# Kim-Dongjun/Soft-Truncation

Measured on AMD Instinct MI355X. Metric: training images/sec (DDPM++ CIFAR-10 32x32), higher is better.
Workload: dtype f32; 1 GPU; DDPM++ (VP) CIFAR-10 32x32, configs/vp/CIFAR10/ddpmpp_nll_st.py (BASELINE configs[1]); per_gpu_batch=128, global_batch=128, parallelism=dp1

## Files before the change

soft-truncation_amd/csrc/conv.hip:

```cpp
#include "igemm.h"
#include "split.h"
#include "stk_fp16.h"
#include "stk_fp16_train.h"

namespace {

using igemm::Cfg;
using igemm::MnMajor;
using igemm::keep_if;
using igemm::strip_row;

typedef __attribute__((address_space(1))) float gfloat;

struct ConvP {
  const float* x1; const float* x2; int C1, C2;
  const float* w; int w_layout;
  const float* bias; const float* temb; int temb_stride; const float* res; float inv_div; int use_div;
  float* y;
  const float* dy; float* dx1; float* dx2; float beta1, beta2, alpha;
  float* part; long part_stride;
  int N, H, W, Cin, Cout, OH, OW, KH, KW, stride, pad, sshift;
  int HW, OHW, taps;
  int ohw_shift, ow_shift;
};
// ... 920 lines not shown
    using A2 = std::conditional_t<X1, x2::ActLoader16<true, TAPS>, x2::ActLoader<true, TAPS>>;
    if (g.dual) hipLaunchKernelGGL((x2::gemm_kernel<A2, E>), g.grid, dim3(256), 0, g.s, g.p, g.q, g.M, g.Ng, g.tm, g.tn, g.nch,
                                   g.chunks_per_split, g.xpart, g.nx);
    else hipLaunchKernelGGL((x2::gemm_kernel<A1, E>), g.grid, dim3(256), 0, g.s, g.p, g.q, g.M, g.Ng, g.tm, g.tn, g.nch,
                            g.chunks_per_split, g.xpart, g.nx);
  } else if (g.halo) {
    if (g.p.W == 64)
      hipLaunchKernelGGL((x2d::gemm_halo_kernel<64, E, 1>), g.grid, dim3(256), 0, g.s, g.p, g.q, g.M, g.Ng, g.tm, g.tn, g.nch / 9, g.xpart, g.nx);
    else if (g.p.W == 32)
      hipLaunchKernelGGL((x2d::gemm_halo_kernel<32, E, 1>), g.grid, dim3(256), 0, g.s, g.p, g.q, g.M, g.Ng, g.tm, g.tn, g.nch / 9, g.xpart, g.nx);
    else
      hipLaunchKernelGGL((x2d::gemm_halo_kernel<16, E, 1>), g.grid, dim3(256), 0, g.s, g.p, g.q, g.M, g.Ng, g.tm, g.tn, g.nch / 9, g.xpart, g.nx);
  } else {
    hipLaunchKernelGGL((x2d::gemm_kernel<TAPS, 128, E>), g.grid, dim3(256), 0, g.s, g.p, g.q, g.M, g.Ng, g.tm, g.tn, g.nch,
                       g.chunks_per_split, g.xpart, g.nx);
  }
}
template <class E>
void split_gemm(const SplitGemm& g) {
  if (g.p.taps == 9) split_gemm_taps<E, 9>(g);
  else split_gemm_taps<E, 1>(g);
}

template <class EP>
int launch_split(ConvP p, const SplitPlan& r0, const float* s1, int S1, const float* s2, int S2, int M, long Ng, int dgrad,
                 void* ws, hipStream_t s, const void* wp_ready, float* amax, const void* planes, const float* planes_amax,
                 bool amax_valid, bool x1) {
  x2::Src q;
  q.s1 = s1; q.s2 = S2 > 0 ? s2 : s1; q.S1 = S1; q.S2 = S2; q.Kc = S1 + S2; q.Mpad = x2::pad128(M); q.taps = p.taps;
  q.pl = static_cast<const unsigned char*>(planes); q.pl_stride = planes ? pl::plane_bytes(p.N, S1, p.HW) : 0;
  const SplitWs lay = split_ws(r0, M, q.Kc, p.taps);
  unsigned char* base = reinterpret_cast<unsigned char*>(((uintptr_t)ws + 255) & ~(uintptr_t)255);
  float* xpart = reinterpret_cast<float*>(base + lay.xpart);
  p.part = reinterpret_cast<float*>(base + lay.part);
  p.part_stride = r0.slab;
  if (amax) xpart = amax + (dgrad ? 2 * x2::NPART : 0);
  if (planes) {
    xpart = const_cast<float*>(planes_amax);
  } else if (!(amax_valid && amax)) {
    hipLaunchKernelGGL(x2::amax_partial_kernel, dim3(x2::NPART), dim3(x2::AMAX_THREADS), 0, s, s1, (long)p.N * S1 * p.HW, xpart);
    if (S2 > 0)
      hipLaunchKernelGGL(x2::amax_partial_kernel, dim3(x2::NPART), dim3(x2::AMAX_THREADS), 0, s, s2, (long)p.N * S2 * p.HW,
                         xpart + x2::NPART);
    STK_CHECK_LAUNCH();
  }
  if (wp_ready) {
    q.wp = static_cast<const unsigned short*>(wp_ready);
  } else {
    x2::WprepDesc one = {};
    one.w = p.w; one.wp = base; one.M = M; one.Kc = q.Kc; one.Mpad = q.Mpad;
    one.taps = p.taps; one.flip = dgrad;
    split_weight_strides(p, dgrad, one.sm, one.sk);
    hipLaunchKernelGGL(x2::wamax_kernel, dim3(x2::WPART, 1), dim3(256), 0, s, nullptr, one);
    hipLaunchKernelGGL(x2::wprep_kernel, dim3((unsigned)stk_cdiv((long)q.Mpad * q.Kc, 256L)), dim3(256), 0, s, nullptr, one);
    STK_CHECK_LAUNCH();
    q.wp = reinterpret_cast<const unsigned short*>(base);
  }
  const int nch = planes && x1 ? p.taps * ((q.Kc / x2::KC + 1) / 2) : p.taps * (q.Kc / x2::KC);
  const SplitPlan r = planes && x1 ? x1_plan(r0, nch) : r0;
  SplitGemm g = {p, q, M, (int)Ng, q.Mpad / 128, stk_cdiv((int)Ng, 128), nch, r.chunks_per_split, xpart,
                 S2 > 0 ? 2 * x2::NPART : x2::NPART, S2 > 0, planes != nullptr, planes && x2d::halo_ok(p, p.taps, r0.splits),
                 dim3(), s};
  g.grid = dim3((unsigned)(g.tm * g.tn * r.splits));
  if (r0.splits == 1) {
    if (x1) split_gemm<OneProduct<EP>>(g);
    else split_gemm<EP>(g);
    STK_CHECK_LAUNCH();
    return STK_OK;
  }
  if (x1) split_gemm<OneProduct<EpSlab>>(g);
  else split_gemm<EpSlab>(g);
  STK_CHECK_LAUNCH();
  launch_slab_sum(p, r.splits, M, Ng, dgrad, s);
  STK_CHECK_LAUNCH();
  return STK_OK;
}

struct SplitWgradPlan { int ok; int splits; int chunks_per_split; long slab; int rows3; };
inline SplitWgradPlan split_wgrad_plan(int C1, int C2, int N, int Cout, int H, int W, int OH, int OW, int KH, int KW,
                                       int stride, int pad) {
  SplitWgradPlan q = {0, 0, 0, 0, 0};
  const int Cin = C1 + C2;
  const long K = (long)N * H * W;
  const int cmax = Cout > C1 ? (Cout > C2 ? Cout : C2) : (C1 > C2 ? C1 : C2);
  if (K * cmax * 4 >= 0x7fffffffL || (C2 > 0 && C1 % 32)) return q;
  const bool pow2 = (W & (W - 1)) == 0 && ((H * W) & (H * W - 1)) == 0;
  const bool geom = (KH == 3 && KW == 3 && pad == 1) || (KH == 1 && KW == 1 && pad == 0);
  if (!geom || stride != 1 || OH != H || OW != W || !pow2 || W < 4 || H * W < 16 || Cin < 64 || Cout < 64 ||
      K > 0x7fffffffL || K % 32)
    return q;
  const int taps = KH * KW;
  q.rows3 = (taps == 9 && W >= 8 && (C2 == 0 || C1 % 16 == 0)) ? 1 : 0;
  const long tiles = q.rows3 ? 3L * stk_cdiv(Cout, 128) * stk_cdiv(Cin, 64)
                             : (long)taps * stk_cdiv(Cout, 128) * stk_cdiv(Cin, 128);
  if (taps == 1 && tiles < 2) return q;
  const long chunks = K / 32;
  constexpr long w1_wgs = 256;
  long splits = (taps == 1 && tiles < 6 ? w1_wgs : 512) / tiles;
  if (splits > chunks / 8) splits = chunks / 8;
  if (splits < 1) splits = 1;
  q.chunks_per_split = (int)((chunks + splits - 1) / splits);
  q.splits = (int)((chunks + q.chunks_per_split - 1) / q.chunks_per_split);
  q.slab = (long)Cout * Cin * taps;
  q.ok = 1;
  return q;
}
template <int FORM>
// ... 43 lines not shown
  q.mode9 = allow9 ? wgrad9_cols(OH, OW, KH, KW) : 0;
  if (q.mode9) {
    const long K = (long)N * OH * OW;
    const long tiles = (long)stk_cdiv(Cout, 128) * stk_cdiv(Cin, 32);
    const long chunks = K / 32;
    long splits = 256 / tiles;
    if (splits > chunks / 16) splits = chunks / 16;
    if (splits < 1) splits = 1;
    const long cps = (chunks + splits - 1) / splits;
    q.big = 1;
    q.k_per_split = (int)(cps * 32);
    q.splits = (int)((K + q.k_per_split - 1) / q.k_per_split);
    q.slab = (long)Cout * Cin * 9;
    return q;
  }
  const int taps = KH * KW;
  const long K = (long)N * OH * OW;
  const long tiles128 = (long)stk_cdiv(Cout, 128) * stk_cdiv(Cin, 128) * taps;
  q.big = (Cout >= 96 && Cin >= 96 && tiles128 >= 9) ? 1 : 0;
  const int T = q.big ? 128 : 64;
  const long tiles = (long)stk_cdiv(Cout, T) * stk_cdiv(Cin, T) * taps;
  const long chunks = (K + 31) / 32;
  long splits = (512 + tiles - 1) / tiles;
  if (splits > chunks / 16) splits = chunks / 16;
  if (splits < 1) splits = 1;
  const long cps = (chunks + splits - 1) / splits;
  q.k_per_split = (int)(cps * 32);
  q.splits = (int)((K + q.k_per_split - 1) / q.k_per_split);
  q.slab = (long)Cout * Cin * taps;
  return q;
}

}

extern "C" {

static int fwd_impl(const float* x1, int C1, const float* x2, int C2, const float* w, int w_layout,
                    const float* bias, const float* temb, int temb_stride, const float* res, float out_div,
                    float* y, int N, int H, int W, int Cout, int OH, int OW, int KH, int KW, int stride, int pad,
                    const void* wp, float* amax, void* ws, long ws_bytes, void* stream, bool x_rec_valid, bool f16x1) {
  if (!x1 || !w || !y || (C2 > 0 && !x2) || out_div == 0.f || (w_layout != 0 && w_layout != 1) ||
      (w_layout == 1 && (KH != 1 || KW != 1)))
    return STK_EINVAL;
  ConvP p = {};
  int rc = fill_common(p, N, H, W, C1, C2, Cout, OH, OW, KH, KW, stride, pad);
  if (rc) return rc;
  p.x1 = x1; p.x2 = C2 > 0 ? x2 : x1; p.w = w; p.w_layout = w_layout; p.bias = bias; p.temb = temb;
  p.temb_stride = temb_stride; p.res = res; p.inv_div = 1.f / out_div; p.use_div = out_div != 1.f; p.y = y;
  const int K = p.Cin * p.taps;
  const long Ng = (long)N * p.OHW;
  const bool big = use_big_tile(Cout, Ng, 1);
  hipStream_t s = (hipStream_t)stream;
  if (thin::geometry_ok(p) && Ng <= 0x7fffffffL) {
    const unsigned nblk = (unsigned)stk_cdiv(Ng, 256L);
    if (C2 == 0 && p.Cin <= 4) {
      thin::Args a = {x1, w, (long)p.Cin * p.taps, (long)p.taps, 0, p.Cin, Cout, p.taps, 0};
      const dim3 grid(nblk, (unsigned)stk_cdiv(Cout, thin::OB));
      if (p.taps == 9) hipLaunchKernelGGL((thin::thin_in_kernel<9>), grid, dim3(256), 0, s, p, a);
      else hipLaunchKernelGGL((thin::thin_in_kernel<1>), grid, dim3(256), 0, s, p, a);
      STK_CHECK_LAUNCH();
      return STK_OK;
    }
    if (Cout <= 4) {
      const unsigned nblk64 = (unsigned)stk_cdiv(Ng, 64L);
      if (p.taps == 9) hipLaunchKernelGGL((thin::thin_out_kernel<9>), dim3(nblk64), dim3(256), 0, s, p, Cout);
      else hipLaunchKernelGGL((thin::thin_out_kernel<1>), dim3(nblk64), dim3(256), 0, s, p, Cout);
      STK_CHECK_LAUNCH();
      return STK_OK;
    }
  }
  const SplitPlan xr = fwd_split_plan(p);
  if (ws && xr.ok && ws_bytes >= split_ws(xr, Cout, p.Cin, p.taps).bytes)
    return launch_split<EpFwd>(p, xr, x1, C1, x2, C2, Cout, Ng, 0, ws, s, wp, amax, nullptr, nullptr, x_rec_valid, f16x1);
  if (wp) return STK_EINVAL;
  if (p.taps == 9) {
    using CB = Cfg<128, 128, 36>; using CS = Cfg<64, 64, 36>;
    if (C2 > 0) {
      if (big) return launch<CB, ConvP, AFwdK<CB>, BFwd<CB, 9, true>, EpFwd>(p, Cout, Ng, K, K, 1, 1, s);
      return launch<CS, ConvP, AFwdK<CS>, BFwd<CS, 9, true>, EpFwd>(p, Cout, Ng, K, K, 1, 1, s);
    }
    if (big) return launch<CB, ConvP, AFwdK<CB>, BFwd<CB, 9, false>, EpFwd>(p, Cout, Ng, K, K, 1, 1, s);
    return launch<CS, ConvP, AFwdK<CS>, BFwd<CS, 9, false>, EpFwd>(p, Cout, Ng, K, K, 1, 1, s);
  }
  using CB = Cfg<128, 128, 32>; using CS = Cfg<64, 64, 32>;
  if (w_layout == 0) {
    if (K % 8 == 0) {
      if (big) return launch<CB, ConvP, AFwdK<CB>, BFwd<CB, 1, true>, EpFwd>(p, Cout, Ng, K, K, 1, 1, s);
      return launch<CS, ConvP, AFwdK<CS>, BFwd<CS, 1, true>, EpFwd>(p, Cout, Ng, K, K, 1, 1, s);
    }
    return launch<CS, ConvP, AFwdGen<CS>, BFwd<CS, 1, true>, EpFwd>(p, Cout, Ng, K, K, 1, 1, s);
  }
  if (big) return launch<CB, ConvP, AFwdNin<CB>, BFwd<CB, 1, true>, EpFwd>(p, Cout, Ng, K, K, 1, 1, s);
  return launch<CS, ConvP, AFwdNin<CS>, BFwd<CS, 1, true>, EpFwd>(p, Cout, Ng, K, K, 1, 1, s);
}

int stk_conv2d_fwd_f32(const float* x1, int C1, const float* x2, int C2, const float* w, int w_layout,
                       const float* bias, const float* temb, int temb_stride, const float* res, float out_div,
                       float* y, int N, int H, int W, int Cout, int OH, int OW, int KH, int KW, int stride, int pad,
                       void* ws, long ws_bytes, void* stream) {
  return stk_conv2d_fwd_wp_f32(x1, C1, x2, C2, w, w_layout, bias, temb, temb_stride, res, out_div, y, N, H, W, Cout, OH, OW,
                               KH, KW, stride, pad, nullptr, nullptr, ws, ws_bytes, stream);
}

int stk_conv2d_fwd_wp_f32(const float* x1, int C1, const float* x2, int C2, const float* w, int w_layout,
                          const float* bias, const float* temb, int temb_stride, const float* res, float out_div,
                          float* y, int N, int H, int W, int Cout, int OH, int OW, int KH, int KW, int stride, int pad,
                          const void* wp, float* amax, void* ws, long ws_bytes, void* stream) {
  return fwd_impl(x1, C1, x2, C2, w, w_layout, bias, temb, temb_stride, res, out_div, y, N, H, W, Cout, OH, OW, KH, KW, stride,
                  pad, wp, amax, ws, ws_bytes, stream, false, false);
}

int stk_conv2d_fwd_rec_f32(const float* x1, int C1, const float* x2, int C2, const float* w, int w_layout,
                           const float* bias, const float* temb, int temb_stride, const float* res, float out_div,
                           float* y, int N, int H, int W, int Cout, int OH, int OW, int KH, int KW, int stride, int pad,
                           const void* wp, float* amax, void* ws, long ws_bytes, void* stream) {
  if (!amax) return STK_EINVAL;
  return fwd_impl(x1, C1, x2, C2, w, w_layout, bias, temb, temb_stride, res, out_div, y, N, H, W, Cout, OH, OW, KH, KW, stride,
                  pad, wp, amax, ws, ws_bytes, stream, true, false);
}

int stk_conv2d_fwd_wp_f16x1(const float* x1, int C1, const float* x2, int C2, const float* w, int w_layout,
                            const float* bias, const float* temb, int temb_stride, const float* res, float out_div,
                            float* y, int N, int H, int W, int Cout, int OH, int OW, int KH, int KW, int stride, int pad,
                            const void* wp, float* amax, void* ws, long ws_bytes, void* stream) {
  return fwd_impl(x1, C1, x2, C2, w, w_layout, bias, temb, temb_stride, res, out_div, y, N, H, W, Cout, OH, OW, KH, KW, stride,
                  pad, wp, amax, ws, ws_bytes, stream, false, true);
}

int stk_conv2d_fwd_rec_f16x1(const float* x1, int C1, const float* x2, int C2, const float* w, int w_layout,
                             const float* bias, const float* temb, int temb_stride, const float* res, float out_div,
                             float* y, int N, int H, int W, int Cout, int OH, int OW, int KH, int KW, int stride, int pad,
                             const void* wp, float* amax, void* ws, long ws_bytes, void* stream) {
  if (!amax) return STK_EINVAL;
  return fwd_impl(x1, C1, x2, C2, w, w_layout, bias, temb, temb_stride, res, out_div, y, N, H, W, Cout, OH, OW, KH, KW, stride,
                  pad, wp, amax, ws, ws_bytes, stream, true, true);
}

static int dgrad_impl(const float* dy, const float* w, int w_layout, float* dx1, int C1, float beta1, float* dx2,
                      int C2, float beta2, float alpha, int N, int H, int W, int Cout, int OH, int OW, int KH,
                      int KW, int stride, int pad, const void* wp, float* amax, void* ws, long ws_bytes,
                      void* stream, bool dy_rec_valid, bool f16x1) {
  if (!dy || !w || (!dx1 && !dx2) || (w_layout != 0 && w_layout != 1) || (w_layout == 1 && (KH != 1 || KW != 1)))
    return STK_EINVAL;
  ConvP p = {};
  int rc = fill_common(p, N, H, W, C1, C2, Cout, OH, OW, KH, KW, stride, pad);
  if (rc) return rc;
  p.dy = dy; p.w = w; p.w_layout = w_layout; p.dx1 = dx1; p.dx2 = C2 > 0 ? dx2 : nullptr;
  p.beta1 = beta1; p.beta2 = beta2; p.alpha = alpha;
  const int Cin = p.Cin;
  const int K = Cout * p.taps;
  const long Ng = (long)N * p.HW;
  const bool big = use_big_tile(Cin, Ng, 1);
  hipStream_t s = (hipStream_t)stream;
  if (thin::geometry_ok(p) && Cout <= 4 && Ng <= 0x7fffffffL) {
    thin::Args a = {dy, w, (long)p.taps, (long)Cin * p.taps, 1, Cout, Cin, p.taps, 1};
    const dim3 grid((unsigned)stk_cdiv(Ng, 256L), (unsigned)stk_cdiv(Cin, thin::OB));
    if (p.taps == 9) hipLaunchKernelGGL((thin::thin_in_kernel<9>), grid, dim3(256), 0, s, p, a);
    else hipLaunchKernelGGL((thin::thin_in_kernel<1>), grid, dim3(256), 0, s, p, a);
    STK_CHECK_LAUNCH();
    return STK_OK;
  }
  const SplitPlan xr = dgrad_split_plan(p);
  if (ws && xr.ok && ws_bytes >= split_ws(xr, Cin, Cout, p.taps).bytes)
    return launch_split<EpDgrad>(p, xr, dy, Cout, nullptr, 0, Cin, Ng, 1, ws, s, wp, amax, nullptr, nullptr, dy_rec_valid, f16x1);
  if (wp) return STK_EINVAL;
  if (p.taps == 9) {
    using CB = Cfg<128, 128, 36>; using CS = Cfg<64, 64, 36>;
    if (big) return launch<CB, ConvP, ADgrad9<CB>, BDgrad<CB, 9>, EpDgrad>(p, Cin, Ng, K, K, 1, 1, s);
    return launch<CS, ConvP, ADgrad9<CS>, BDgrad<CS, 9>, EpDgrad>(p, Cin, Ng, K, K, 1, 1, s);
  }
  using CB = Cfg<128, 128, 32>; using CS = Cfg<64, 64, 32>;
  if (w_layout == 0) {
    if (big) return launch<CB, ConvP, ADgrad1<CB>, BDgrad<CB, 1>, EpDgrad>(p, Cin, Ng, K, K, 1, 1, s);
    return launch<CS, ConvP, ADgrad1<CS>, BDgrad<CS, 1>, EpDgrad>(p, Cin, Ng, K, K, 1, 1, s);
  }
  if (K % 8 != 0) return launch<CS, ConvP, ADgradNinGen<CS>, BDgrad<CS, 1>, EpDgrad>(p, Cin, Ng, K, K, 1, 1, s);
  if (big) return launch<CB, ConvP, ADgradNin<CB>, BDgrad<CB, 1>, EpDgrad>(p, Cin, Ng, K, K, 1, 1, s);
  return launch<CS, ConvP, ADgradNin<CS>, BDgrad<CS, 1>, EpDgrad>(p, Cin, Ng, K, K, 1, 1, s);
}

int stk_conv2d_dgrad_f32(const float* dy, const float* w, int w_layout, float* dx1, int C1, float beta1, float* dx2,
                         int C2, float beta2, float alpha, int N, int H, int W, int Cout, int OH, int OW, int KH,
                         int KW, int stride, int pad, void* ws, long ws_bytes, void* stream) {
  return stk_conv2d_dgrad_wp_f32(dy, w, w_layout, dx1, C1, beta1, dx2, C2, beta2, alpha, N, H, W, Cout, OH, OW, KH, KW, stride,
                                 pad, nullptr, nullptr, ws, ws_bytes, stream);
}

int stk_conv2d_dgrad_wp_f32(const float* dy, const float* w, int w_layout, float* dx1, int C1, float beta1, float* dx2,
                            int C2, float beta2, float alpha, int N, int H, int W, int Cout, int OH, int OW, int KH,
                            int KW, int stride, int pad, const void* wp, float* amax, void* ws, long ws_bytes,
                            void* stream) {
  return dgrad_impl(dy, w, w_layout, dx1, C1, beta1, dx2, C2, beta2, alpha, N, H, W, Cout, OH, OW, KH, KW, stride, pad, wp,
                    amax, ws, ws_bytes, stream, false, false);
}

int stk_conv2d_dgrad_rec_f32(const float* dy, const float* w, int w_layout, float* dx1, int C1, float beta1, float* dx2,
                             int C2, float beta2, float alpha, int N, int H, int W, int Cout, int OH, int OW, int KH,
                             int KW, int stride, int pad, const void* wp, float* amax, void* ws, long ws_bytes,
                             void* stream) {
  if (!amax) return STK_EINVAL;
  return dgrad_impl(dy, w, w_layout, dx1, C1, beta1, dx2, C2, beta2, alpha, N, H, W, Cout, OH, OW, KH, KW, stride, pad, wp,
                    amax, ws, ws_bytes, stream, true, false);
}

int stk_conv2d_dgrad_wp_f16x1(const float* dy, const float* w, int w_layout, float* dx1, int C1, float beta1, float* dx2,
                              int C2, float beta2, float alpha, int N, int H, int W, int Cout, int OH, int OW, int KH,
                              int KW, int stride, int pad, const void* wp, float* amax, void* ws, long ws_bytes,
                              void* stream) {
  return dgrad_impl(dy, w, w_layout, dx1, C1, beta1, dx2, C2, beta2, alpha, N, H, W, Cout, OH, OW, KH, KW, stride, pad, wp,
                    amax, ws, ws_bytes, stream, false, true);
}
// ... 307 lines not shown
  return wgrad_pl_impl(xpl, xrec, dypl, dyrec, dw, alpha, ws, ws_bytes, N, H, W, Cin, Cout, wgs, stream, true);
}

int stk_conv2d_variant(int dir, int C1, int C2, int N, int H, int W, int Cout, int OH, int OW, int KH, int KW,
                       int stride, int pad, int w_layout) {
  ConvP p = {};
  if (fill_common(p, N, H, W, C1, C2, Cout, OH, OW, KH, KW, stride, pad)) return -1;
  const int Cin = C1 + C2;
  p.w_layout = w_layout;
  if (dir == 0) {
    const long Ng = (long)N * p.OHW;
    if (thin::geometry_ok(p) && ((C2 == 0 && Cin <= 4) || Cout <= 4)) return 4;
    if (fwd_split_plan(p).ok) return 5;
    return use_big_tile(Cout, Ng, 1) && !(p.taps == 1 && w_layout == 0 && (Cin % 8)) ? 1 : 0;
  }
  if (dir == 1) {
    const long Ng = (long)N * p.HW;
    if (thin::geometry_ok(p) && Cout <= 4) return 4;
    if (dgrad_split_plan(p).ok) return 5;
    return use_big_tile(Cin, Ng, 1) && !(p.taps == 1 && w_layout == 1 && (Cout % 8)) ? 1 : 0;
  }
  if (thin::geometry_ok(p) && ((C2 == 0 && Cin <= 4) || Cout <= 4)) return 4;
  if (split_wgrad_plan(C1, C2, N, Cout, H, W, OH, OW, KH, KW, stride, pad).ok) return 5;
  const bool can9 = stride == 1 && pad == 1 && C2 == 0 && OH == H && OW == W && w_layout == 0;
  const WgradPlan q = wgrad_plan(Cin, N, Cout, OH, OW, KH, KW, can9);
  return q.mode9 ? 3 : q.big;
}

long stk_conv2d_wp_bytes(int dir, int C1, int C2, int N, int H, int W, int Cout, int KH, int KW, int stride, int pad) {
  if (dir != 0 && dir != 1) return 0;
  if (stk_conv2d_variant(dir, C1, C2, N, H, W, Cout, H, W, KH, KW, stride, pad, 0) != 5) return 0;
  const int Cin = C1 + C2;
  return dir == 0 ? x2::wp_bytes(Cout, Cin, KH * KW) : x2::wp_bytes(Cin, Cout, KH * KW);
}

long stk_conv2d_wp_desc(int dir, const float* w, int w_layout, int Cin, int Cout, int KH, int KW, void* wp,
                        StkWprepDesc* out) {
  if (!w || !wp || !out || (dir != 0 && dir != 1) || (w_layout != 0 && w_layout != 1) || Cin <= 0 || Cout <= 0 ||
      (KH * KW != 9 && KH * KW != 1) || (w_layout == 1 && KH * KW != 1) || ((uintptr_t)wp & 255))
    return STK_EINVAL;
  ConvP p = {};
  p.Cin = Cin; p.Cout = Cout; p.taps = KH * KW; p.w_layout = w_layout;
  long sm, sk;
  split_weight_strides(p, dir, sm, sk);
  out->w = w; out->wp = wp; out->sm = sm; out->sk = sk;
  out->M = dir ? Cin : Cout; out->Kc = dir ? Cout : Cin; out->Mpad = x2::pad128(out->M); out->taps = p.taps;
  out->flip = dir; out->reserved = 0;
  return (long)out->Mpad * out->Kc;
}

int stk_conv2d_wprep_batch(const StkWprepDesc* descs_dev, int n, long max_items, void* stream) {
  static_assert(sizeof(StkWprepDesc) == sizeof(x2::WprepDesc), "descriptor layout");
  if (!descs_dev || n <= 0 || max_items <= 0 || n > 65535) return STK_EINVAL;
  const dim3 grid((unsigned)stk_cdiv(max_items, 256L), (unsigned)n);
  const x2::WprepDesc* d = reinterpret_cast<const x2::WprepDesc*>(descs_dev);
  hipLaunchKernelGGL(x2::wamax_kernel, dim3(x2::WPART, (unsigned)n), dim3(256), 0, (hipStream_t)stream, d, x2::WprepDesc{});
  hipLaunchKernelGGL(x2::wprep_kernel, grid, dim3(256), 0, (hipStream_t)stream, d, x2::WprepDesc{});
  STK_CHECK_LAUNCH();
  return STK_OK;
}

long stk_conv2d_fwd_ws_bytes(int C1, int C2, int N, int H, int W, int Cout, int KH, int KW, int stride, int pad) {
  ConvP p = {};
  if (fill_common(p, N, H, W, C1, C2, Cout, H, W, KH, KW, stride, pad)) return 0;
  return split_ws(fwd_split_plan(p), Cout, C1 + C2, p.taps).bytes;
}

long stk_conv2d_dgrad_ws_bytes(int C1, int C2, int N, int H, int W, int Cout, int KH, int KW, int stride, int pad) {
  ConvP p = {};
  if (fill_common(p, N, H, W, C1, C2, Cout, H, W, KH, KW, stride, pad)) return 0;
  return split_ws(dgrad_split_plan(p), C1 + C2, Cout, p.taps).bytes;
}

long stk_conv2d_wgrad_ws_bytes(int C1, int C2, int N, int Cout, int OH, int OW, int KH, int KW) {
  const WgradPlan a = wgrad_plan(C1 + C2, N, Cout, OH, OW, KH, KW, true);
  const WgradPlan b = wgrad_plan(C1 + C2, N, Cout, OH, OW, KH, KW, false);
  const SplitWgradPlan x = split_wgrad_plan(C1, C2, N, Cout, OH, OW, OH, OW, KH, KW, 1, KH == 3 ? 1 : 0);
  const long na = (long)a.splits * a.slab, nb = (long)b.splits * b.slab, nx = x.ok ? (long)x.splits * x.slab : 0;
  long m = na > nb ? na : nb;
  if (C2 == 0 && C1 <= 4) { const long t = (long)thin::wgrad_slabs(N, (long)OH * OW, Cout) * Cout * C1 * KH * KW; m = t > m ? t : m; }
  if (Cout <= 4) { const long t = (long)thin::wgrad_slabs(N, (long)OH * OW, C1 + C2) * Cout * (C1 + C2) * KH * KW; m = t > m ? t : m; }
  return (m > nx ? m : nx) * 4 + 256 + 256 + 3L * x2::NPART * 4;
}

int stk_gemm_f32(const float* A, long sam, long sak, long sab, const float* B, long sbk, long sbn, long sbb, float* C,
                 long scm, long scn, long scb, const float* bias, int bias_mode, int M, int N, int K, int batch,
                 float alpha, float beta, void* stream) {
  if (!A || !B || !C || M <= 0 || N <= 0 || K <= 0 || batch <= 0 || (bias_mode && !bias) || bias_mode < 0 ||
      bias_mode > 2)
    return STK_EINVAL;
  GemmP p;
  p.A = A; p.sam = sam; p.sak = sak; p.sab = sab; p.B = B; p.sbk = sbk; p.sbn = sbn; p.sbb = sbb;
  p.C = C; p.scm = scm; p.scn = scn; p.scb = scb; p.bias = bias; p.bias_mode = bias_mode;
  p.M = M; p.N = N; p.K = K; p.alpha = alpha; p.beta = beta;
  const bool ak = sak == 1 && (K % 8) == 0;
  const bool bk = sbk == 1 && sbn != 1 && (K % 8) == 0;
  const bool big = use_big_tile(M, N, batch);
  hipStream_t s = (hipStream_t)stream;
  using CB = Cfg<128, 128, 32>; using CS = Cfg<64, 64, 32>;
#define STK_GEMM_CASE(AK, BK)                                                                              \
  if (ak == AK && bk == BK) {                                                                              \
    if (big) return launch<CB, GemmP, GA<CB, AK>, GB<CB, BK>, EpGemm>(p, M, N, K, K, 1, batch, s);         \
    return launch<CS, GemmP, GA<CS, AK>, GB<CS, BK>, EpGemm>(p, M, N, K, K, 1, batch, s);                  \
  }
  STK_GEMM_CASE(true, true)
  STK_GEMM_CASE(true, false)
  STK_GEMM_CASE(false, true)
// ... 7 lines not shown
```

soft-truncation_amd/csrc/conv_thin.h:

```cpp
#pragma once

namespace thin {

constexpr int MAXK = 36;
constexpr int OB = 32;

struct Args {
  const float* thin;
  const float* w;
  long so, sc;
  int flip, CT, OUT, taps;
  int dgrad;
};

__device__ __forceinline__ unsigned tap_mask(int y, int x, int H, int W, int taps) {
  if (taps == 1) return 1u;
  unsigned m = 0;
#pragma unroll
  for (int t = 0; t < 9; ++t) {
    const int iy = y + t / 3 - 1, ix = x + t % 3 - 1;
    if (iy >= 0 && iy < H && ix >= 0 && ix < W) m |= 1u << t;
  }
  return m;
}

template <int TAPS>
__global__ __launch_bounds__(256) void thin_in_kernel(ConvP p, Args a) {
  __shared__ __attribute__((aligned(16))) float w_s[OB * MAXK];
  const int K = a.CT * TAPS;
  const int o0 = blockIdx.y * OB, no = min(OB, a.OUT - o0);
  for (int i = threadIdx.x; i < no * 4 * TAPS; i += 256) {
    const int o = i / (4 * TAPS), k = i - o * 4 * TAPS, c = k / TAPS, t = k - c * TAPS;
    w_s[o * MAXK + k] = k < K ? a.w[(long)(o0 + o) * a.so + c * a.sc + (a.flip ? TAPS - 1 - t : t)] : 0.f;
  }
  const long n = (long)blockIdx.x * 256 + threadIdx.x;
  const bool live = n < (long)p.N * p.HW;
  const int b = live ? (int)(n / p.HW) : 0, hw = live ? (int)(n - (long)b * p.HW) : 0;
  const int y = hw / p.W, x = hw - y * p.W;
  const unsigned mask = live ? tap_mask(y, x, p.H, p.W, TAPS) : 0u;
  float xv[MAXK];
#pragma unroll
  for (int k = 0; k < MAXK; ++k) xv[k] = 0.f;
  {
    const float* base = a.thin + (long)b * a.CT * p.HW + hw;
#pragma unroll
    for (int c = 0; c < 4; ++c)
#pragma unroll
      for (int t = 0; t < TAPS; ++t) {
        const bool ok = c < a.CT && ((mask >> t) & 1u);
        const int off = TAPS == 9 ? (t / 3 - 1) * p.W + (t % 3 - 1) : 0;
        const float v = base[ok ? (long)c * p.HW + off : 0];
        xv[c * TAPS + t] = ok ? v : 0.f;
      }
  }
  __syncthreads();
  if (!live) return;
  const float inv_div = p.inv_div;
  for (int o = 0; o < no; ++o) {
    const float4* wr = reinterpret_cast<const float4*>(w_s + o * MAXK);
    float acc = 0.f;
#pragma unroll
    for (int k4 = 0; k4 < (4 * TAPS + 3) / 4; ++k4) {
      const float4 wv = wr[k4];
      acc += wv.x * xv[4 * k4] + wv.y * xv[4 * k4 + 1] + wv.z * xv[4 * k4 + 2] + wv.w * xv[4 * k4 + 3];
    }
    const int oc = o0 + o;
    if (!a.dgrad) {
      const long idx = ((long)b * a.OUT + oc) * p.HW + hw;
      float v = acc;
      if (p.bias) v += p.bias[oc];
      if (p.temb) v += p.temb[(long)b * p.temb_stride + oc];
      if (p.res) v += p.res[idx];
      if (p.use_div) v *= inv_div;
      p.y[idx] = v;
    } else {
      float* d; float beta;
      if (oc < p.C1) { d = p.dx1 ? p.dx1 + ((long)b * p.C1 + oc) * p.HW + hw : nullptr; beta = p.beta1; }
      else { d = p.dx2 ? p.dx2 + ((long)b * p.C2 + (oc - p.C1)) * p.HW + hw : nullptr; beta = p.beta2; }
      if (d) *d = (beta != 0.f ? beta * *d : 0.f) + p.alpha * acc;
    }
  }
}

template <int TAPS>
__global__ __launch_bounds__(256) void thin_out_kernel(ConvP p, int CO) {
  __shared__ __attribute__((aligned(16))) float w_s[128 * 9 * 4];
  __shared__ float red[4][4][64];
  const int lane = threadIdx.x & 63, q = threadIdx.x >> 6;
  const long n = (long)blockIdx.x * 64 + lane;
  const bool live = n < (long)p.N * p.HW;
  const int b = live ? (int)(n / p.HW) : 0, hw = live ? (int)(n - (long)b * p.HW) : 0;
  const int y = hw / p.W, x = hw - y * p.W;
  const unsigned mask = live ? tap_mask(y, x, p.H, p.W, TAPS) : 0u;
  int off[TAPS];
#pragma unroll
  for (int t = 0; t < TAPS; ++t) off[t] = ((mask >> t) & 1u) ? (TAPS == 9 ? (t / 3 - 1) * p.W + (t % 3 - 1) : 0) : 0;
  float acc[4] = {0.f, 0.f, 0.f, 0.f};
  for (int c0 = 0; c0 < p.Cin; c0 += 128) {
    const int nc = min(128, p.Cin - c0);
    __syncthreads();
    for (int i = threadIdx.x; i < 4 * nc * TAPS; i += 256) {
      const int o = i & 3, r = i >> 2;
      w_s[r * 4 + o] = o < CO ? p.w[((long)o * p.Cin + c0) * TAPS + r] : 0.f;
    }
    __syncthreads();
    const int ce = min(nc, q * 32 + 32);
#pragma unroll 2
    for (int c = q * 32; c < ce; ++c) {
      const int ci = c0 + c;
      const float* plane = ci < p.C1 ? p.x1 + ((long)b * p.C1 + ci) * p.HW + hw
                                     : p.x2 + ((long)b * p.C2 + (ci - p.C1)) * p.HW + hw;
      float v[TAPS];
#pragma unroll
      for (int t = 0; t < TAPS; ++t) v[t] = plane[off[t]];
#pragma unroll
      for (int t = 0; t < TAPS; ++t) {
        const float xv = ((mask >> t) & 1u) ? v[t] : 0.f;
        const float4 wv = *reinterpret_cast<const float4*>(w_s + (c * TAPS + t) * 4);
        acc[0] += wv.x * xv; acc[1] += wv.y * xv; acc[2] += wv.z * xv; acc[3] += wv.w * xv;
      }
    }
  }
#pragma unroll
  for (int o = 0; o < 4; ++o) red[q][o][lane] = acc[o];
  __syncthreads();
  if (!live || q >= CO) return;
  const int o = q;
  float v = ((red[0][o][lane] + red[1][o][lane]) + red[2][o][lane]) + red[3][o][lane];
  const long idx = ((long)b * CO + o) * p.HW + hw;
  if (p.bias) v += p.bias[o];
  if (p.temb) v += p.temb[(long)b * p.temb_stride + o];
  if (p.res) v += p.res[idx];
// ... 33 lines not shown
    for (int c = 0; c < CTT; ++c)
#pragma unroll
      for (int t = 0; t < TAPS; ++t) {
        const bool ok = c < a.CT && ((mask >> t) & 1u);
        const int off = TAPS == 9 ? (t / 3 - 1) * p.W + (t % 3 - 1) : 0;
        const float v = tb[ok ? (long)c * p.HW + off : 0];
        pv[c * TAPS + t] = ok ? v : 0.f;
      }
#pragma unroll
    for (int j = 0; j < 4; ++j) {
      const int bc = bc0 + j;
      if (bc < BC) {
        const float* bp = bc < a.B1 ? a.b1 + ((long)n * a.B1 + bc) * p.HW : a.b2 + ((long)n * a.B2 + (bc - a.B1)) * p.HW;
        const float v = live ? bp[hw] : 0.f;
#pragma unroll
        for (int k = 0; k < KK; ++k) acc[j][k] += v * pv[k];
      }
    }
  }
#pragma unroll
  for (int j = 0; j < 4; ++j) {
#pragma unroll
    for (int k = 0; k < KK; ++k) red[wv][k * 65 + lane] = acc[j][k];
    __syncthreads();
    if (lane < KK) {
      float sum = 0.f;
      for (int i = 0; i < 64; ++i) sum += red[wv][lane * 65 + i];
      wsum[wv][j * KK + lane] = sum;
    }
    __syncthreads();
  }
  if (tid < 4 * KK) {
    const int j = tid / KK, k = tid - j * KK, c = k / TAPS, t = k - c * TAPS, bc = bc0 + j;
    if (bc < BC && c < a.CT) {
      const float total = ((wsum[0][tid] + wsum[1][tid]) + wsum[2][tid]) + wsum[3][tid];
      const long idx = a.head ? ((long)(TAPS - 1 - t) * a.CT + c) * BC + bc : ((long)t * BC + bc) * a.CT + c;
      a.part[(long)blockIdx.x * a.slab + idx] = total;
    }
  }
}

inline int wgrad_slabs(int N, long HW, int BC) {
  const long items = (long)N * ((HW + 255) / 256);
  long s = 1024 / ((BC + 3) / 4);
  if (s < 1) s = 1;
  return (int)(s < items ? s : items);
}

inline bool geometry_ok(const ConvP& p) {
  return p.stride == 1 && p.OH == p.H && p.OW == p.W && ((p.taps == 9 && p.pad == 1) || (p.taps == 1 && p.pad == 0)) &&
         p.w_layout == 0;
}

}
```

soft-truncation_amd/csrc/conv_x2.h:

```cpp
#pragma once

typedef _Float16 halfx8 __attribute__((ext_vector_type(8)));

namespace x2 {

using split2::pow2_scale_of;
using split2::pack_h2;
using split2::lo_part;

constexpr int KC = 32;
constexpr int PITCH = 80;
constexpr int PLANE = 128 * PITCH;
constexpr int OPER = 2 * PLANE;
constexpr int LDS_BYTES = 2 * OPER;
constexpr int NPART = 256;
constexpr int HEADER = 256;

struct Src {
  const float* s1; const float* s2; int S1, S2;
  const unsigned short* wp; int Mpad; int Kc;
  int taps;
  const unsigned char* pl; long pl_stride;
};

// ... 49 lines not shown
struct LateAmax {
  float m;
  __device__ __forceinline__ void load(const float* __restrict__ part, int count, int tid) {
    m = part[tid];
    if (count > NPART) m = fmaxf(m, part[NPART + tid]);
  }
  __device__ __forceinline__ float reduce(float* red, int tid) {
    const float v = wave_max(m);
    if ((tid & 63) == 0) red[tid >> 6] = v;
    __syncthreads();
    return fmaxf(fmaxf(red[0], red[1]), fmaxf(red[2], red[3]));
  }
};

struct WprepDesc {
  const float* w; unsigned char* wp; long sm, sk; int M, Kc, Mpad, taps, flip, reserved;
};
constexpr int WPART = 16;
__global__ __launch_bounds__(256) void wamax_kernel(const WprepDesc* __restrict__ descs, WprepDesc one) {
  __shared__ float red[4];
  const WprepDesc d = descs ? descs[blockIdx.y] : one;
  const long n = (long)d.M * d.Kc * d.taps;
  float m = 0.f;
  if ((reinterpret_cast<uintptr_t>(d.w) & 15) == 0) {
    const float4* w4 = reinterpret_cast<const float4*>(d.w);
    const long n4 = n >> 2;
    for (long i = (long)blockIdx.x * 1024 + threadIdx.x; i < n4; i += (long)WPART * 1024) {
      float4 v[4];
#pragma unroll
      for (int u = 0; u < 4; ++u) {
        const long j = i + 256 * u;
        v[u] = j < n4 ? w4[j] : make_float4(0.f, 0.f, 0.f, 0.f);
      }
#pragma unroll
      for (int u = 0; u < 4; ++u)
        m = fmaxf(m, fmaxf(fmaxf(fabsf(v[u].x), fabsf(v[u].y)), fmaxf(fabsf(v[u].z), fabsf(v[u].w))));
    }
    if (blockIdx.x == 0 && threadIdx.x < (n & 3)) m = fmaxf(m, fabsf(d.w[(n4 << 2) + threadIdx.x]));
  } else {
    for (long i = (long)blockIdx.x * 256 + threadIdx.x; i < n; i += (long)WPART * 256) m = fmaxf(m, fabsf(d.w[i]));
  }
  m = wave_max(m);
  if ((threadIdx.x & 63) == 0) red[threadIdx.x >> 6] = m;
  __syncthreads();
  if (threadIdx.x == 0) reinterpret_cast<float*>(d.wp)[blockIdx.x] = fmaxf(fmaxf(red[0], red[1]), fmaxf(red[2], red[3]));
}
__device__ __forceinline__ float weight_scale(const void* header) {
  const float* h = static_cast<const float*>(header);
  float m = 0.f;
#pragma unroll
  for (int i = 0; i < WPART; ++i) m = fmaxf(m, h[i]);
  return pow2_scale_of(m);
}
__global__ __launch_bounds__(256) void wprep_kernel(const WprepDesc* __restrict__ descs, WprepDesc one) {
  const WprepDesc d = descs ? descs[blockIdx.y] : one;
  const long total = (long)d.Mpad * d.Kc;
  const long i = (long)blockIdx.x * 256 + threadIdx.x;
  if (i >= total) return;
  const float s = weight_scale(d.wp);
  unsigned short* out = reinterpret_cast<unsigned short*>(d.wp + HEADER);
  const int kl = (int)(i & 31);
  const long rest = i >> 5;
  const int row = (int)(rest % d.Mpad), cc = (int)(rest / d.Mpad), k = cc * 32 + kl;
  const long plane = (long)d.taps * d.Mpad * d.Kc;
  const float* src = d.w + (row < d.M ? row * d.sm + k * d.sk : 0);
  for (int t = 0; t < d.taps; ++t) {
    const float a = row < d.M ? s * src[d.flip ? d.taps - 1 - t : t] : 0.f;
    const _Float16 h0 = (_Float16)a, h1 = (_Float16)(a - (float)h0);
    const long o = (((long)cc * d.taps + t) * d.Mpad + row) * 32 + kl;
    out[o] = __builtin_bit_cast(unsigned short, h0);
    out[plane + o] = __builtin_bit_cast(unsigned short, h1);
  }
}
inline long wp_bytes(int M, int Kc, int taps) { return HEADER + 2L * taps * pad128(M) * Kc * 2; }

template <bool X1>
struct Split16X {
  unsigned pk[2][8];
  __device__ __forceinline__ void st(int g, const float (&r)[16], float s, unsigned char* tile, int row, int k0,
                                     unsigned okm = 0xffffu) {
    if (g < 8) {
      const float v0 = s * igemm::keep_if(r[2 * g], okm, 2 * g), v1 = s * igemm::keep_if(r[2 * g + 1], okm, 2 * g + 1);
      pk[0][g] = pack_h2(v0, v1);
      if (!X1) pk[1][g] = pack_h2(lo_part(v0), lo_part(v1));
    } else if (g < 12) {
      const int sp = (g - 8) >> 1, h = (g - 8) & 1;
      if (X1 && sp) return;
      *reinterpret_cast<u32x4*>(tile + sp * PLANE + row * PITCH + k0 * 2 + h * 16) =
          u32x4{pk[sp][4 * h], pk[sp][4 * h + 1], pk[sp][4 * h + 2], pk[sp][4 * h + 3]};
    }
  }
};
using Split16 = Split16X<false>;

struct WpLoader {
  __amdgpu_buffer_rsrc_t rs; unsigned voff, plane2, chunk2; int row, seg;
  u32x4 r[4];
  __device__ __forceinline__ void init(const Src& q, int m0, int tid) {
    row = tid >> 2; seg = tid & 3;
    plane2 = (unsigned)q.taps * q.Mpad * q.Kc * 2u;
    chunk2 = (unsigned)q.Mpad * KC * 2u;
    rs = make_rsrc(reinterpret_cast<const unsigned char*>(q.wp) + HEADER, 2L * plane2);
    voff = ((unsigned)(m0 + row) * KC + seg * 8) * 2u;
  }
  __device__ __forceinline__ void ld(int g, int c) {
    if (g >= 4) return;
    r[g] = __builtin_bit_cast(u32x4, __builtin_amdgcn_raw_buffer_load_b128(
                                         rs, (int)voff, (int)((unsigned)c * chunk2 + (g >> 1) * plane2 + (g & 1) * 64u * KC * 2u), 0));
  }
  __device__ __forceinline__ void st(int g, unsigned char* t) {
    if (g < 4) *reinterpret_cast<u32x4*>(t + (g >> 1) * PLANE + (row + 64 * (g & 1)) * PITCH + seg * 16) = r[g];
  }
};

template <bool DUAL, int TAPS, bool X1>
struct ActLoaderT {
  __amdgpu_buffer_rsrc_t rs1, rs2;
  int nl, kg, tb1, tb2; unsigned mask; float scale;
  float r[16]; Split16X<X1> sp;
  __device__ __forceinline__ void init(const ConvP& p, const Src& q, int n0, int tid, float s) {
    nl = tid & 127;
    kg = __builtin_amdgcn_readfirstlane(tid >> 7);
    rs1 = make_rsrc(q.s1, (long)p.N * q.S1 * p.HW * 4);
    rs2 = make_rsrc(q.s2, (long)p.N * (DUAL ? q.S2 : q.S1) * p.HW * 4);
    mask = 0; tb1 = 0; tb2 = 0; scale = s;
// ... 562 lines not shown
```

Measured before the change: 3491 images/s.

## Tile weight-prep through LDS and compute four pixels per thread in thin convs

The weight-prep kernel now stages a 32-row by 32-k tile in shared memory, reading it with vectorized float4 loads and writing the fp16 hi/lo split planes as 16-byte stores. Before, each thread did strided scalar reads and 2-byte writes. The thin-channel conv kernel is templated on the channel count, and each thread now computes a run of four adjacent output pixels from a register-held 3x6 input window. Outputs use float4 stores, and there are 16 output channels per block. This is meant to cut redundant input loads and narrow memory transactions, at the cost of more register pressure and more template variants.

```diff
diff --git a/soft-truncation_amd/csrc/conv.hip b/soft-truncation_amd/csrc/conv.hip
--- a/soft-truncation_amd/csrc/conv.hip
+++ b/soft-truncation_amd/csrc/conv.hip
@@ -996,7 +996,7 @@
     one.taps = p.taps; one.flip = dgrad;
     split_weight_strides(p, dgrad, one.sm, one.sk);
     hipLaunchKernelGGL(x2::wamax_kernel, dim3(x2::WPART, 1), dim3(256), 0, s, nullptr, one);
-    hipLaunchKernelGGL(x2::wprep_kernel, dim3((unsigned)stk_cdiv((long)q.Mpad * q.Kc, 256L)), dim3(256), 0, s, nullptr, one);
+    hipLaunchKernelGGL(x2::wprep_kernel, dim3((unsigned)stk_cdiv((long)q.Mpad * q.Kc, (long)x2::WPREP_ITEMS)), dim3(256), 0, s, nullptr, one);
     STK_CHECK_LAUNCH();
     q.wp = reinterpret_cast<const unsigned short*>(base);
   }
@@ -1146,12 +1146,9 @@
   const bool big = use_big_tile(Cout, Ng, 1);
   hipStream_t s = (hipStream_t)stream;
   if (thin::geometry_ok(p) && Ng <= 0x7fffffffL) {
-    const unsigned nblk = (unsigned)stk_cdiv(Ng, 256L);
     if (C2 == 0 && p.Cin <= 4) {
       thin::Args a = {x1, w, (long)p.Cin * p.taps, (long)p.taps, 0, p.Cin, Cout, p.taps, 0};
-      const dim3 grid(nblk, (unsigned)stk_cdiv(Cout, thin::OB));
-      if (p.taps == 9) hipLaunchKernelGGL((thin::thin_in_kernel<9>), grid, dim3(256), 0, s, p, a);
-      else hipLaunchKernelGGL((thin::thin_in_kernel<1>), grid, dim3(256), 0, s, p, a);
+      thin::launch_in(p, a, s);
       STK_CHECK_LAUNCH();
       return STK_OK;
     }
@@ -1248,9 +1245,7 @@
   hipStream_t s = (hipStream_t)stream;
   if (thin::geometry_ok(p) && Cout <= 4 && Ng <= 0x7fffffffL) {
     thin::Args a = {dy, w, (long)p.taps, (long)Cin * p.taps, 1, Cout, Cin, p.taps, 1};
-    const dim3 grid((unsigned)stk_cdiv(Ng, 256L), (unsigned)stk_cdiv(Cin, thin::OB));
-    if (p.taps == 9) hipLaunchKernelGGL((thin::thin_in_kernel<9>), grid, dim3(256), 0, s, p, a);
-    else hipLaunchKernelGGL((thin::thin_in_kernel<1>), grid, dim3(256), 0, s, p, a);
+    thin::launch_in(p, a, s);
     STK_CHECK_LAUNCH();
     return STK_OK;
   }
@@ -1664,7 +1659,7 @@
 int stk_conv2d_wprep_batch(const StkWprepDesc* descs_dev, int n, long max_items, void* stream) {
   static_assert(sizeof(StkWprepDesc) == sizeof(x2::WprepDesc), "descriptor layout");
   if (!descs_dev || n <= 0 || max_items <= 0 || n > 65535) return STK_EINVAL;
-  const dim3 grid((unsigned)stk_cdiv(max_items, 256L), (unsigned)n);
+  const dim3 grid((unsigned)stk_cdiv(max_items, (long)x2::WPREP_ITEMS), (unsigned)n);
   const x2::WprepDesc* d = reinterpret_cast<const x2::WprepDesc*>(descs_dev);
   hipLaunchKernelGGL(x2::wamax_kernel, dim3(x2::WPART, (unsigned)n), dim3(256), 0, (hipStream_t)stream, d, x2::WprepDesc{});
   hipLaunchKernelGGL(x2::wprep_kernel, grid, dim3(256), 0, (hipStream_t)stream, d, x2::WprepDesc{});
diff --git a/soft-truncation_amd/csrc/conv_thin.h b/soft-truncation_amd/csrc/conv_thin.h
--- a/soft-truncation_amd/csrc/conv_thin.h
+++ b/soft-truncation_amd/csrc/conv_thin.h
@@ -2,8 +2,7 @@
 
 namespace thin {
 
-constexpr int MAXK = 36;
-constexpr int OB = 32;
+constexpr int OB4 = 16;
 
 struct Args {
   const float* thin;
@@ -24,60 +23,108 @@
   return m;
 }
 
-template <int TAPS>
+template <int TAPS, int CTT>
 __global__ __launch_bounds__(256) void thin_in_kernel(ConvP p, Args a) {
-  __shared__ __attribute__((aligned(16))) float w_s[OB * MAXK];
-  const int K = a.CT * TAPS;
-  const int o0 = blockIdx.y * OB, no = min(OB, a.OUT - o0);
-  for (int i = threadIdx.x; i < no * 4 * TAPS; i += 256) {
-    const int o = i / (4 * TAPS), k = i - o * 4 * TAPS, c = k / TAPS, t = k - c * TAPS;
-    w_s[o * MAXK + k] = k < K ? a.w[(long)(o0 + o) * a.so + c * a.sc + (a.flip ? TAPS - 1 - t : t)] : 0.f;
-  }
-  const long n = (long)blockIdx.x * 256 + threadIdx.x;
-  const bool live = n < (long)p.N * p.HW;
-  const int b = live ? (int)(n / p.HW) : 0, hw = live ? (int)(n - (long)b * p.HW) : 0;
-  const int y = hw / p.W, x = hw - y * p.W;
-  const unsigned mask = live ? tap_mask(y, x, p.H, p.W, TAPS) : 0u;
-  float xv[MAXK];
-#pragma unroll
-  for (int k = 0; k < MAXK; ++k) xv[k] = 0.f;
+  constexpr int K = CTT * TAPS, KP = (K + 3) / 4 * 4;
+  constexpr int ROWS = TAPS == 9 ? 3 : 1, TX = TAPS == 9 ? 3 : 1, COLS = 3 + TX;
+  __shared__ __attribute__((aligned(16))) float w_s[OB4 * KP];
+  const int o0 = blockIdx.y * OB4, no = min(OB4, a.OUT - o0);
+  for (int i = threadIdx.x; i < no * KP; i += 256) {
+    const int o = i / KP, k = i - o * KP, c = k / TAPS, t = k - c * TAPS;
+    w_s[i] = (k < K && c < a.CT) ? a.w[(long)(o0 + o) * a.so + c * a.sc + (a.flip ? TAPS - 1 - t : t)] : 0.f;
+  }
+  const int WQ = (p.W + 3) >> 2;
+  const long per_img = (long)p.H * WQ;
+  const long r = (long)blockIdx.x * 256 + threadIdx.x;
+  const bool live = r < (long)p.N * per_img;
+  const int b = live ? (int)(r / per_img) : 0, rem = live ? (int)(r - (long)b * per_img) : 0;
+  const int y = rem / WQ, x0 = (rem - y * WQ) * 4;
+  float xv[CTT][ROWS][COLS];
   {
-    const float* base = a.thin + (long)b * a.CT * p.HW + hw;
-#pragma unroll
-    for (int c = 0; c < 4; ++c)
-#pragma unroll
-      for (int t = 0; t < TAPS; ++t) {
-        const bool ok = c < a.CT && ((mask >> t) & 1u);
-        const int off = TAPS == 9 ? (t / 3 - 1) * p.W + (t % 3 - 1) : 0;
-        const float v = base[ok ? (long)c * p.HW + off : 0];
-        xv[c * TAPS + t] = ok ? v : 0.f;
-      }
+    const float* base = a.thin + (long)b * a.CT * p.HW;
+#pragma unroll
+    for (int c = 0; c < CTT; ++c)
+#pragma unroll
+      for (int ry = 0; ry < ROWS; ++ry)
+#pragma unroll
+        for (int cx = 0; cx < COLS; ++cx) {
+          const int iy = y + (TAPS == 9 ? ry - 1 : 0), ix = x0 + cx - (TAPS == 9 ? 1 : 0);
+          const bool ok = live && c < a.CT && iy >= 0 && iy < p.H && ix >= 0 && ix < p.W;
+          const float v = base[ok ? (long)c * p.HW + iy * p.W + ix : 0];
+          xv[c][ry][cx] = ok ? v : 0.f;
+        }
   }
   __syncthreads();
   if (!live) return;
   const float inv_div = p.inv_div;
+  const int hw0 = y * p.W + x0, npx = min(4, p.W - x0);
+  const bool v4 = (p.W & 3) == 0 && ((reinterpret_cast<uintptr_t>(p.y) | reinterpret_cast<uintptr_t>(p.res) |
+                                      reinterpret_cast<uintptr_t>(p.dx1) | reinterpret_cast<uintptr_t>(p.dx2)) & 15) == 0;
   for (int o = 0; o < no; ++o) {
-    const float4* wr = reinterpret_cast<const float4*>(w_s + o * MAXK);
-    float acc = 0.f;
-#pragma unroll
-    for (int k4 = 0; k4 < (4 * TAPS + 3) / 4; ++k4) {
+    const float4* wr = reinterpret_cast<const float4*>(w_s + o * KP);
+    float wk[KP];
+#pragma unroll
+    for (int k4 = 0; k4 < KP / 4; ++k4) {
       const float4 wv = wr[k4];
-      acc += wv.x * xv[4 * k4] + wv.y * xv[4 * k4 + 1] + wv.z * xv[4 * k4 + 2] + wv.w * xv[4 * k4 + 3];
-    }
+      wk[4 * k4] = wv.x; wk[4 * k4 + 1] = wv.y; wk[4 * k4 + 2] = wv.z; wk[4 * k4 + 3] = wv.w;
+    }
+    float acc[4] = {0.f, 0.f, 0.f, 0.f};
+#pragma unroll
+    for (int g = 0; g < KP / 4; ++g)
+#pragma unroll
+      for (int px = 0; px < 4; ++px) {
+        float xk[4];
+#pragma unroll
+        for (int u = 0; u < 4; ++u) {
+          const int k = 4 * g + u < K ? 4 * g + u : 0, c = k / TAPS, t = k - c * TAPS;
+          xk[u] = 4 * g + u < K ? xv[c][t / TX][px + t % TX] : 0.f;
+        }
+        float sum = wk[4 * g + 1] * xk[1];
+        sum = __builtin_fmaf(wk[4 * g], xk[0], sum);
+        if (4 * g + 2 < K) sum = __builtin_fmaf(wk[4 * g + 2], xk[2], sum);
+        if (4 * g + 3 < K) sum = __builtin_fmaf(wk[4 * g + 3], xk[3], sum);
+        acc[px] = acc[px] + sum;
+      }
     const int oc = o0 + o;
     if (!a.dgrad) {
-      const long idx = ((long)b * a.OUT + oc) * p.HW + hw;
-      float v = acc;
-      if (p.bias) v += p.bias[oc];
-      if (p.temb) v += p.temb[(long)b * p.temb_stride + oc];
-      if (p.res) v += p.res[idx];
-      if (p.use_div) v *= inv_div;
-      p.y[idx] = v;
+      const long idx = ((long)b * a.OUT + oc) * p.HW + hw0;
+      const float bs = p.bias ? p.bias[oc] : 0.f, tm = p.temb ? p.temb[(long)b * p.temb_stride + oc] : 0.f;
+      float rs[4] = {0.f, 0.f, 0.f, 0.f};
+      if (p.res) {
+        if (v4) { const float4 q = *reinterpret_cast<const float4*>(p.res + idx); rs[0] = q.x; rs[1] = q.y; rs[2] = q.z; rs[3] = q.w; }
+        else {
+#pragma unroll
+          for (int px = 0; px < 4; ++px) if (px < npx) rs[px] = p.res[idx + px];
+        }
+      }
+      float v[4];
+#pragma unroll
+      for (int px = 0; px < 4; ++px) {
+        v[px] = acc[px];
+        if (p.bias) v[px] += bs;
+        if (p.temb) v[px] += tm;
+        if (p.res) v[px] += rs[px];
+        if (p.use_div) v[px] *= inv_div;
+      }
+      if (v4) *reinterpret_cast<float4*>(p.y + idx) = make_float4(v[0], v[1], v[2], v[3]);
+      else {
+#pragma unroll
+        for (int px = 0; px < 4; ++px) if (px < npx) p.y[idx + px] = v[px];
+      }
     } else {
       float* d; float beta;
-      if (oc < p.C1) { d = p.dx1 ? p.dx1 + ((long)b * p.C1 + oc) * p.HW + hw : nullptr; beta = p.beta1; }
-      else { d = p.dx2 ? p.dx2 + ((long)b * p.C2 + (oc - p.C1)) * p.HW + hw : nullptr; beta = p.beta2; }
-      if (d) *d = (beta != 0.f ? beta * *d : 0.f) + p.alpha * acc;
+      if (oc < p.C1) { d = p.dx1 ? p.dx1 + ((long)b * p.C1 + oc) * p.HW + hw0 : nullptr; beta = p.beta1; }
+      else { d = p.dx2 ? p.dx2 + ((long)b * p.C2 + (oc - p.C1)) * p.HW + hw0 : nullptr; beta = p.beta2; }
+      if (!d) continue;
+      if (v4) {
+        float4 q = make_float4(0.f, 0.f, 0.f, 0.f);
+        if (beta != 0.f) { q = *reinterpret_cast<const float4*>(d); q.x *= beta; q.y *= beta; q.z *= beta; q.w *= beta; }
+        *reinterpret_cast<float4*>(d) = make_float4(q.x + p.alpha * acc[0], q.y + p.alpha * acc[1], q.z + p.alpha * acc[2],
+                                                    q.w + p.alpha * acc[3]);
+      } else {
+#pragma unroll
+        for (int px = 0; px < 4; ++px) if (px < npx) d[px] = (beta != 0.f ? beta * d[px] : 0.f) + p.alpha * acc[px];
+      }
     }
   }
 }
@@ -217,4 +264,13 @@
          p.w_layout == 0;
 }
 
-}
+
+inline void launch_in(const ConvP& p, const Args& a, hipStream_t s) {
+  const long runs = (long)p.N * p.H * ((p.W + 3) / 4);
+  const dim3 grid((unsigned)stk_cdiv(runs, 256L), (unsigned)stk_cdiv(a.OUT, OB4));
+  if (p.taps == 1) hipLaunchKernelGGL((thin_in_kernel<1, 4>), grid, dim3(256), 0, s, p, a);
+  else if (a.CT == 3) hipLaunchKernelGGL((thin_in_kernel<9, 3>), grid, dim3(256), 0, s, p, a);
+  else hipLaunchKernelGGL((thin_in_kernel<9, 4>), grid, dim3(256), 0, s, p, a);
+}
+
+}
diff --git a/soft-truncation_amd/csrc/conv_x2.h b/soft-truncation_amd/csrc/conv_x2.h
--- a/soft-truncation_amd/csrc/conv_x2.h
+++ b/soft-truncation_amd/csrc/conv_x2.h
@@ -125,25 +125,92 @@
   for (int i = 0; i < WPART; ++i) m = fmaxf(m, h[i]);
   return pow2_scale_of(m);
 }
+constexpr int WT = 32;
+constexpr int WPITCH = 36;
+template <int TAPS>
+__device__ __forceinline__ void wprep_tile(const WprepDesc& d, float* st) {
+  constexpr int RUN = 32 * TAPS;
+  constexpr int NV = RUN / 4 / 8;
+  static_assert(WT == 32 && RUN == NV * 4 * 8, "tile geometry: 32 runs, eight threads each");
+  const int tid = threadIdx.x;
+  const int rtiles = d.Mpad / WT;
+  const int cc = blockIdx.x / rtiles, r0 = (blockIdx.x - cc * rtiles) * WT;
+  const float s = weight_scale(d.wp);
+  if (r0 < d.M) {
+    const bool rows_inner = d.sk != TAPS && d.sm == TAPS;
+    const long so = rows_inner ? d.sk : d.sm, sa = rows_inner ? d.sm : d.sk;
+    const float* base = d.w + (long)r0 * d.sm + (long)cc * 32 * d.sk;
+    const bool vec = sa == TAPS && (so & 3) == 0 && (reinterpret_cast<uintptr_t>(base) & 15) == 0;
+    const int rows = d.M - r0;
+    const int outer = tid >> 3;
+    float4 v[NV];
+    if (vec) {
+#pragma unroll
+      for (int i = 0; i < NV; ++i) {
+        const int inner = ((tid & 7) + 8 * i) * 4;
+        const float* src = base + outer * so + inner;
+        const int last_row = rows_inner ? (inner + 3) / TAPS : outer;
+        if (last_row < rows) {
+          v[i] = *reinterpret_cast<const float4*>(src);
+        } else {
+          float q[4];
+#pragma unroll
+          for (int j = 0; j < 4; ++j) q[j] = (rows_inner ? (inner + j) / TAPS : outer) < rows ? src[j] : 0.f;
+          v[i] = make_float4(q[0], q[1], q[2], q[3]);
+        }
+      }
+    } else {
+#pragma unroll
+      for (int i = 0; i < NV; ++i) {
+        float q[4];
+#pragma unroll
+        for (int j = 0; j < 4; ++j) {
+          const int inner = ((tid & 7) + 8 * i) * 4 + j, a = inner / TAPS;
+          q[j] = (rows_inner ? a : outer) < rows ? base[outer * so + a * sa + (inner - a * TAPS)] : 0.f;
+        }
+        v[i] = make_float4(q[0], q[1], q[2], q[3]);
+      }
+    }
+#pragma unroll
+    for (int i = 0; i < NV; ++i) {
+      const float q[4] = {v[i].x, v[i].y, v[i].z, v[i].w};
+#pragma unroll
+      for (int j = 0; j < 4; ++j) {
+        const int inner = ((tid & 7) + 8 * i) * 4 + j, a = inner / TAPS, tp = inner - a * TAPS;
+        const int row = rows_inner ? a : outer, k = rows_inner ? outer : a, t = d.flip ? TAPS - 1 - tp : tp;
+        st[(t * WT + row) * WPITCH + k] = q[j];
+      }
+    }
+  }
+  __syncthreads();
+  const long plane = (long)TAPS * d.Mpad * d.Kc * 2;
+  unsigned char* out = d.wp + HEADER;
+  for (int j = tid; j < TAPS * WT * 4; j += 256) {
+    const int t = j / (WT * 4), rem = j - t * (WT * 4), row = rem >> 2, kq = rem & 3;
+    float x[8];
+    if (r0 + row < d.M) {
+      const float4 lo4 = *reinterpret_cast<const float4*>(st + (t * WT + row) * WPITCH + kq * 8);
+      const float4 hi4 = *reinterpret_cast<const float4*>(st + (t * WT + row) * WPITCH + kq * 8 + 4);
+      x[0] = s * lo4.x; x[1] = s * lo4.y; x[2] = s * lo4.z; x[3] = s * lo4.w;
+      x[4] = s * hi4.x; x[5] = s * hi4.y; x[6] = s * hi4.z; x[7] = s * hi4.w;
+    } else {
+#pragma unroll
+      for (int u = 0; u < 8; ++u) x[u] = 0.f;
+    }
+    u32x4 hi, lo;
+    split2::split8(x, hi, lo);
+    const long o = ((((long)cc * TAPS + t) * d.Mpad + r0 + row) * 32 + kq * 8) * 2;
+    *reinterpret_cast<u32x4*>(out + o) = hi;
+    *reinterpret_cast<u32x4*>(out + plane + o) = lo;
+  }
+}
+constexpr int WPREP_ITEMS = WT * 32;
 __global__ __launch_bounds__(256) void wprep_kernel(const WprepDesc* __restrict__ descs, WprepDesc one) {
+  __shared__ __attribute__((aligned(16))) float st[9 * WT * WPITCH];
   const WprepDesc d = descs ? descs[blockIdx.y] : one;
-  const long total = (long)d.Mpad * d.Kc;
-  const long i = (long)blockIdx.x * 256 + threadIdx.x;
-  if (i >= total) return;
-  const float s = weight_scale(d.wp);
-  unsigned short* out = reinterpret_cast<unsigned short*>(d.wp + HEADER);
-  const int kl = (int)(i & 31);
-  const long rest = i >> 5;
-  const int row = (int)(rest % d.Mpad), cc = (int)(rest / d.Mpad), k = cc * 32 + kl;
-  const long plane = (long)d.taps * d.Mpad * d.Kc;
-  const float* src = d.w + (row < d.M ? row * d.sm + k * d.sk : 0);
-  for (int t = 0; t < d.taps; ++t) {
-    const float a = row < d.M ? s * src[d.flip ? d.taps - 1 - t : t] : 0.f;
-    const _Float16 h0 = (_Float16)a, h1 = (_Float16)(a - (float)h0);
-    const long o = (((long)cc * d.taps + t) * d.Mpad + row) * 32 + kl;
-    out[o] = __builtin_bit_cast(unsigned short, h0);
-    out[plane + o] = __builtin_bit_cast(unsigned short, h1);
-  }
+  if ((long)blockIdx.x >= (long)(d.Mpad / WT) * (d.Kc / 32)) return;
+  if (d.taps == 9) wprep_tile<9>(d, st);
+  else wprep_tile<1>(d, st);
 }
 inline long wp_bytes(int M, int Kc, int taps) { return HEADER + 2L * taps * pad128(M) * Kc * 2; }
 
```

After: 3505 images/s (median of 6 runs). About the same (+0.4%).
